# MaximEremenko/WebGPU-FFT

Measured on AMD Instinct MI355X. Metric: 1D c2c f32 GPoints/s at N=2^20 batch=4096, higher is better.
Workload: dtype f32

## Files before the change

webgpu-fft_amd/csrc/kern_regtile.hpp:

```cpp
#pragma once
#include "kern_xcd_real.hpp"
#include "kern_xcd_res.hpp"

namespace mi355 {

#ifndef MI355_RT_NT_OUT
#define MI355_RT_NT_OUT 0
#endif
#ifndef MI355_RT_EXP_SKIP_LAST
#define MI355_RT_EXP_SKIP_LAST 0
#endif
#ifndef MI355_RT_EXP_ALIGN
#define MI355_RT_EXP_ALIGN 0
#endif
#ifndef MI355_RT_EXP_ASC
#define MI355_RT_EXP_ASC 0
#endif
#ifndef MI355_RT_ONLY_PHASE
#define MI355_RT_ONLY_PHASE 0
#endif
#ifndef MI355_RT_NT_IN
#define MI355_RT_NT_IN MI355_XCD_NT
#endif
constexpr bool RT_NT_OUT = MI355_RT_NT_OUT != 0, RT_NT_IN = MI355_RT_NT_IN != 0;
// ... 305 lines not shown
#pragma unroll
        for (int q = 0; q < 16; ++q) rt_separate_store(wt, (unsigned)(32 + 64 * q), N2, wb[q], wb[31 - q]);
      }
      __syncthreads();
    }
    xcd_arrive(&f.ctl->bar[gslot][0]);
    if (!xcd_wait(&f.ctl->bar[gslot][0], (k + 1u) * gsize, f.spin_limit, f.sticky_error, &s_words[6])) return;
    cf* const po = f.out + tr * (f.out_pitch - MI355_RT_EXP_ALIGN);
    constexpr int sh = 0;
    for (unsigned tile = rank; tile < (MI355_RT_ONLY_PHASE == 1 ? 0u : (ROWS + 15) / 16 - MI355_RT_EXP_SKIP_LAST); tile += gsize) {
      cf v[64], v0[32], v1[32];
      const int r0 = (int)(tile * 16u) - sh;
      const int line = t >> 5, u = t & 31;
      {
        const int rr = r0 + line;
        const unsigned row = rr < 0 ? 0u : (rr < (int)ROWS ? (unsigned)rr : ROWS - 1);
        const cf* p = W + (size_t)row * N2 + u;
#pragma unroll
        for (int m = 0; m < 64; ++m) v[m] = p[32 * m];
        rt_fourstep(v, f, row, u);
      }
      rt_dft64(v, v0, v1);
      cf w[32];
      const int rl = t & 15, jj = t >> 4;
      const int k1s = r0 + rl;
      const unsigned k1 = (unsigned)k1s;
      const bool live = k1s >= 0 && k1s < (int)ROWS, edge = k1 == 0 || k1 == N1 / 2;
      rt_exchange_first(v0, v1, w, xb, line, u, rl, jj);
#pragma unroll
      for (int c = 0; c < 2; ++c) {
        const int j2 = jj + 32 * c;
        if (c == 1) rt_exchange_second(w, xb, rl, jj);
        rt_stage2(w, tw2, j2);
        if (f.scale != 1.0f) {
#pragma unroll
          for (int q = 0; q < 32; ++q) w[q] = w[q] * f.scale;
        }
        const unsigned kb = k1 + N1 * (unsigned)j2;
        if (live) {
#pragma unroll
          for (int q = 0; q < 16; ++q) st_stream<RT_NT_OUT>(po + (kb + (unsigned)(64 * q) * N1), w[q]);
        }
        if (live && !edge) {
#pragma unroll
          for (int q = 16; q < 32; ++q) { cf mm; mm.x = w[q].x; mm.y = -w[q].y; st_stream<RT_NT_OUT>(po + (NREAL - MI355_RT_EXP_ALIGN - (MI355_RT_EXP_ASC ? kb + 15u - 2u * (unsigned)rl : kb) - (unsigned)(64 * q) * N1), mm); }
        }
        if (c == 0 && k1 == 0 && jj == 0) st_stream<RT_NT_OUT>(po + NREAL / 2, w[16]);
      }
      __syncthreads();
    }
    if (!two_slots) {
      xcd_arrive(&f.ctl->bar[gslot][1]);
      if (!xcd_wait(&f.ctl->bar[gslot][1], (k + 1u) * gsize, f.spin_limit, f.sticky_error, &s_words[6])) return;
    }
  }
}
template <int N1_> struct XcdRtR2cCfgN { static constexpr int THREADS = RtCfg::THREADS, LDS_BYTES = XcdRtCfg<N1_, false>::LDS_BYTES; };

template <int N1_>
__global__ void __launch_bounds__(RtCfg::THREADS) fft_xcd_rt_c2r_kernel(const XcdFusedArgs f) {
  static_assert(N1_ == 2048 || N1_ == 1024, "2048 x 2048, or 1024 x 2048 with pass A on LDS-resident 16 x 1024 tiles (the packing then walks the LDS image)");
  using XC = XcdRtCfg<N1_, false>;
  using CA = typename XC::CA;
  MI_SMEM_DECL(smem);
  cf* xb = reinterpret_cast<cf*>(smem);
  cf* tw_a = xb + XC::DATA;
  cf* tw2 = tw_a + XC::TW_A;
  unsigned* s_words = reinterpret_cast<unsigned*>(tw2 + RtCfg::TW2_ELEMS);
  const int t = threadIdx.x;
  if constexpr (!XC::A_RT) { for (int i = t; i < XC::TW_A; i += RtCfg::THREADS) tw_a[i] = f.tw_a[i]; }
  for (int i = t; i < RtCfg::TW2_ELEMS; i += RtCfg::THREADS) tw2[i] = f.tw_b[i];
  if (!xcd_register(f.ctl, f.split, f.spin_limit, f.sticky_error, s_words)) return;
  const unsigned gslot = s_words[0], rank = s_words[1], gsize = s_words[2], gidx = s_words[4], groups = s_words[5];

  constexpr int N1 = N1_, N2 = 2048, COLS = N2 / 2 + 1;
  LineArgs aa{};
  aa.tw = f.tw_a; aa.num_tiles = (COLS + 15) / 16; aa.num_lines = COLS; aa.out_S = 16; aa.out_outer_stride = 0; aa.scale = 1.0f; aa.fs_group = 1;
  constexpr size_t wsize = (size_t)(N1 / 2) * N2;
  const bool two_slots = f.slots != 1u;
  cf* const W0 = f.wslots + (size_t)((two_slots ? 2u : 1u) * gslot) * wsize;
  const auto root = [&](unsigned m) { return cmul(f.tw_hi[m >> f.fs_shift], f.tw_lo[m & f.fs_lo_mask]); };
  unsigned k = 0;
  for (long long tr = gidx; tr < f.num_transforms; tr += groups, ++k) {
    cf* const W = W0 + (size_t)(two_slots ? (k & 1u) : 0u) * wsize;
    const cf* const X = f.in + tr * f.in_pitch;
    if constexpr (!XC::A_RT) {
      for (unsigned tile = rank; tile < (COLS + 15) / 16; tile += gsize) {
        cf v[CA::E];
        {
          const int line = t & 15, u = t >> 4;
          const int n2r = (int)(tile * 16u) + line, n2 = n2r > N2 / 2 ? N2 / 2 : n2r;
          const int up = u * N2 + n2;
          const int lo = n2 ? (N1 - 1 - u) * N2 + (N2 - n2) : (N1 - u) * N2;
#pragma unroll
          for (int q = 0; q < 32; ++q) {
            const int step = q * (N1 / 32) * N2;
            if (q < 16) { const cf x = X[up + step]; v[q] = cf{x.x, -x.y}; }
            else v[q] = X[lo - step];
          }
        }
        stage_compute_write<CA, 0>(v, aa, tile, t, xb, tw_a, nullptr);
        __syncthreads();
        stage_read<CA, 1>(v, aa, tile, t, xb);
        __syncthreads();
        stage_compute_write<CA, 1, false, true>(v, aa, tile, t, xb, tw_a, nullptr);
        __syncthreads();
        for (int p = t; p < (N1 / 2) * 16; p += RtCfg::THREADS) {
          const int i = p >> 4, c = p & 15;
          const int n2r = (int)(tile * 16u) + c;
          if (n2r > N2 / 2) continue;
          const cf a = cmul(xb[(2 * i) * 16 + c], root((unsigned)(2 * i) * (unsigned)n2r));
          const cf b = cmul(xb[(2 * i + 1) * 16 + c], root((unsigned)(2 * i + 1) * (unsigned)n2r));
          W[(size_t)i * N2 + n2r] = cf{a.x - b.y, a.y + b.x};
          if (n2r >= 1 && n2r < N2 / 2) W[(size_t)i * N2 + (N2 - n2r)] = cf{a.x + b.y, b.x - a.y};
        }
        __syncthreads();
      }
    } else
    for (unsigned tile = rank; tile < (COLS + 15) / 16; tile += gsize) {
      const int line = t & 15, i = t >> 4;
      cf v[64], v0[32], v1[32];
      const int n2r = (int)(tile * 16u) + line;
      const int n2 = n2r > N2 / 2 ? N2 / 2 : n2r;
      {
        const int up = i * N2 + n2;
        const int lo = n2 ? (N1 - 1 - i) * N2 + (N2 - n2) : (N1 - i) * N2;
#pragma unroll
        for (int m = 0; m < 32; ++m) { const cf x = X[up + (32 * m) * N2]; v[m] = cf{x.x, -x.y}; }
#pragma unroll
        for (int m = 32; m < 64; ++m) v[m] = X[lo - (32 * m) * N2];
      }
      rt_dft64(v, v0, v1);
      cf wa[32], wb[32];
      rt_exchange_first<true>(v0, v1, wa, xb, line, i, line, i);
      rt_stage2(wa, tw2, 2 * i);
      rt_exchange_second(wb, xb, line, i);
      rt_stage2(wb, tw2, 2 * i + 1);
      const bool live = n2r <= N2 / 2, mirror = live && n2r >= 1 && n2r < N2 / 2;
      const cf step = root(64u * (unsigned)n2);
      cf* const pd = W + (unsigned)i * N2 + (unsigned)n2;
      cf* const pm = W + (unsigned)i * N2 + (unsigned)(N2 - n2);
#pragma unroll
      for (int g = 0; g < 32; g += 8) {
        cf ra = root((unsigned)(2 * i + 64 * g) * (unsigned)n2), rb = root((unsigned)(2 * i + 1 + 64 * g) * (unsigned)n2);
#pragma unroll
        for (int q = g; q < g + 8; ++q) {
          const cf a = cmul(wa[q], ra), b = cmul(wb[q], rb);
          if (live) pd[(unsigned)(32 * q) * N2] = cf{a.x - b.y, a.y + b.x};
          if (mirror) pm[(unsigned)(32 * q) * N2] = cf{a.x + b.y, b.x - a.y};
          ra = cmul(ra, step); rb = cmul(rb, step);
        }
      }
      __syncthreads();
    }
    xcd_arrive(&f.ctl->bar[gslot][0]);
    if (!xcd_wait(&f.ctl->bar[gslot][0], (k + 1u) * gsize, f.spin_limit, f.sticky_error, &s_words[6])) return;
    cf* const y = f.out + tr * f.out_pitch;
    for (unsigned tile = rank; tile < (N1 / 2) / 16; tile += gsize) {
      cf v[64];
      rt_load_rows(v, W, tile * 16u, t);
      rt_finish_rows<false, RT_NT_OUT, false>(v, y, f, N1 / 2, tile * 16u, f.scale, t, xb, tw2, [](cf (&)[64]) {});
    }
    if (!two_slots) {
      xcd_arrive(&f.ctl->bar[gslot][1]);
      if (!xcd_wait(&f.ctl->bar[gslot][1], (k + 1u) * gsize, f.spin_limit, f.sticky_error, &s_words[6])) return;
    }
  }
}

#ifndef MI355_HX_WAVES
#define MI355_HX_WAVES 4
#endif
struct HxCfg {
  static constexpr int N = 1024, T = 16, THREADS = 512;
  static constexpr int HALF_ELEMS = T * 32 * 16;
  static constexpr int TW1_ELEMS = 31 * 32;
  static constexpr int LDS_BYTES = (HALF_ELEMS + TW1_ELEMS) * 8 + 64;
};

MI_DEV void hx_exchange(const cf (&v)[32], cf (&w)[32], cf* xb, int line, int u, int rl, int jj, bool first) {
  const int wb = u * 256 + ((line + u) & 15);
  const int rb = (jj & 15) * 16;
  if (first) {
#pragma unroll
    for (int q = 0; q < 16; ++q) xb[wb + q * 16] = v[q];
    __syncthreads();
#pragma unroll
    for (int uu = 0; uu < 32; ++uu) w[uu] = xb[uu * 256 + rb + ((rl + uu) & 15)];
    __syncthreads();
#pragma unroll
    for (int q = 0; q < 16; ++q) xb[wb + q * 16] = v[16 + q];
    __syncthreads();
    __syncthreads();
  } else {
#pragma unroll
    for (int q = 0; q < 16; ++q) xb[wb + q * 16] = v[q];
    __syncthreads();
    __syncthreads();
#pragma unroll
    for (int q = 0; q < 16; ++q) xb[wb + q * 16] = v[16 + q];
    __syncthreads();
#pragma unroll
    for (int uu = 0; uu < 32; ++uu) w[uu] = xb[uu * 256 + rb + ((rl + uu) & 15)];
    __syncthreads();
  }
}

template <bool INV>
__global__ void __launch_bounds__(HxCfg::THREADS, MI355_HX_WAVES) fft_xcd_hx_kernel(const XcdFusedArgs f) {
  MI_SMEM_DECL(smem);
  cf* xb = reinterpret_cast<cf*>(smem);
  cf* tw1 = xb + HxCfg::HALF_ELEMS;
  unsigned* s_words = reinterpret_cast<unsigned*>(tw1 + HxCfg::TW1_ELEMS);
  const int t = threadIdx.x;
  for (int i = t; i < HxCfg::TW1_ELEMS; i += HxCfg::THREADS) tw1[i] = f.tw_a[i];
  if (!xcd_register(f.ctl, f.split, f.spin_limit, f.sticky_error, s_words)) return;
  const unsigned gslot = s_words[0], rank = s_words[1], gsize = s_words[2], gidx = s_words[4], groups = s_words[5];
  constexpr unsigned N1 = 1024, N2 = 1024, NT = 64;
  const bool two_slots = f.slots != 1u;
  cf* const W0 = f.wslots + (size_t)((two_slots ? 2u : 1u) * gslot) * (size_t)f.N;
  const int cl = t & 15, cu = t >> 4;
  const int rl_ = t >> 5, ru = t & 31;
  const bool first = MI_UNIFORM_U32((unsigned)t >> 8) == 0u;
  const auto root = [&](unsigned m) { return cmul(f.tw_hi[m >> f.fs_shift], f.tw_lo[m & f.fs_lo_mask]); };
  unsigned k = 0;
  for (long long tr = gidx; tr < f.num_transforms; tr += groups, ++k) {
    cf* const W = W0 + (size_t)(two_slots ? (k & 1u) : 0u) * (size_t)f.N;
    const cf* const x = f.in + tr * f.in_pitch;
    for (unsigned tile = rank; tile < NT; tile += gsize) {
      cf v[32], w[32];
      {
        const cf* p = x + tile * 16u;
        const unsigned voff = (unsigned)cu * N2 + (unsigned)cl;
#pragma unroll
        for (int q = 0; q < 32; ++q) v[q] = cswap_if<INV>(ld_stream<RT_NT_IN>(sgpr_base(p + (unsigned)(32 * q) * N2) + voff));
      }
      fft_radix<32>(v);
      hx_exchange(v, w, xb, cl, cu, cl, cu, first);
      { int ti = cu; MI_OPAQUE_LANE_INT(ti);
#pragma unroll
      for (int q = 1; q < 32; ++q) w[q] = cmul(w[q], tw1[(q - 1) * 32 + ti]); }
      fft_radix<32>(w);
      cf* po = W + tile * 16u;
      const unsigned so = (unsigned)cu * N2 + (unsigned)cl;
#pragma unroll
      for (int q = 0; q < 32; ++q) *(sgpr_base(po + (unsigned)(32 * q) * N2) + so) = w[q];
    }
    xcd_arrive(&f.ctl->bar[gslot][0]);
    if (!xcd_wait(&f.ctl->bar[gslot][0], (k + 1u) * gsize, f.spin_limit, f.sticky_error, &s_words[6])) return;
    cf* const y = f.out + tr * f.out_pitch;
    for (unsigned tile = rank; tile < NT; tile += gsize) {
      cf v[32], w[32];
      {
        const unsigned k1 = tile * 16u + (unsigned)rl_;
        const cf* p = W + (size_t)(tile * 16u) * N2;
        const unsigned lo = (unsigned)rl_ * N2 + (unsigned)ru;
#pragma unroll
        for (int q = 0; q < 32; ++q) v[q] = *(sgpr_base(p + 32 * q) + lo);
        const cf step = root(k1 * 32u);
#pragma unroll
        for (int g = 0; g < 4; ++g) {
          cf r = root(k1 * (unsigned)(ru + 256 * g));
#pragma unroll
          for (int j = 0; j < 8; ++j) { v[8 * g + j] = cmul(v[8 * g + j], r); if (j < 7) r = cmul(r, step); }
        }
      }
      fft_radix<32>(v);
      hx_exchange(v, w, xb, rl_, ru, cl, cu, first);
      { int ti = cu; MI_OPAQUE_LANE_INT(ti);
#pragma unroll
      for (int q = 1; q < 32; ++q) w[q] = cmul(w[q], tw1[(q - 1) * 32 + ti]); }
      fft_radix<32>(w);
      cf* po = y + tile * 16u;
      const unsigned so = (unsigned)cu * N1 + (unsigned)cl;
#pragma unroll
      for (int q = 0; q < 32; ++q) {
        cf r = w[q];
        if (f.scale != 1.0f) r = r * f.scale;
        st_stream<XCD_NT>(sgpr_base(po + (unsigned)(32 * q) * N1) + so, cswap_if<INV>(r));
      }
    }
    if (!two_slots) {
      xcd_arrive(&f.ctl->bar[gslot][1]);
      if (!xcd_wait(&f.ctl->bar[gslot][1], (k + 1u) * gsize, f.spin_limit, f.sticky_error, &s_words[6])) return;
    }
  }
}

#ifndef MI355_RT1K_NT_OUT
#define MI355_RT1K_NT_OUT MI355_XCD_NT
#endif
#ifndef MI355_RT1K_NT_IN
#define MI355_RT1K_NT_IN MI355_RT_NT_IN
#endif
#ifndef MI355_RT1K_TW_FENCE
#define MI355_RT1K_TW_FENCE 8
#endif
#ifndef MI355_RT1K_PREFETCH
#define MI355_RT1K_PREFETCH 0
#endif
#ifndef MI355_RT1K_W_NT
#define MI355_RT1K_W_NT 0
#endif
template <int T_ = 32> struct Rt1kCfgT {
  static constexpr int N = 1024, T = T_, THREADS = 16 * T_;
  static constexpr int HALF_ELEMS = T * 32 * 16;
  static constexpr int TW1_ELEMS = 31 * 32;
  static constexpr int LDS_BYTES = (HALF_ELEMS + TW1_ELEMS) * 8 + 64;
};
using Rt1kCfg = Rt1kCfgT<32>;
template <int T = 32> MI_DEV int rt1k_slot(int line, int pl, int u) { return u * (16 * T) + pl * T + ((line + (u >> 1)) & (T - 1)); }

template <int T = 32, class Mid>
MI_DEV void rt1k_exchange(const cf (&va)[32], const cf (&vb)[32], cf (&w)[32], cf* xb, int line, int ua, int ub, int cl, int h, Mid&& mid) {
  const int wa = rt1k_slot<T>(line, 0, ua), wb2 = rt1k_slot<T>(line, 0, ub);
#pragma unroll
  for (int p = 0; p < 16; ++p) { xb[wa + p * T] = va[p]; xb[wb2 + p * T] = vb[p]; }
  __syncthreads();
#pragma unroll
  for (int uu = 0; uu < 32; ++uu) w[uu] = xb[uu * (16 * T) + h * T + ((cl + (uu >> 1)) & (T - 1))];
  __syncthreads();
#pragma unroll
  for (int p = 0; p < 16; ++p) { xb[wa + p * T] = va[16 + p]; xb[wb2 + p * T] = vb[16 + p]; }
  __syncthreads();
  MI_SCHED_FENCE();
  mid();
  MI_SCHED_FENCE();
#pragma unroll
  for (int uu = 0; uu < 32; ++uu) w[uu] = xb[uu * (16 * T) + h * T + ((cl + (uu >> 1)) & (T - 1))];
}

template <bool INV, int T = 32, bool VIEW = false, int N1_ = 1024>
__global__ void __launch_bounds__(Rt1kCfgT<T>::THREADS, 2) fft_xcd_rt1k_kernel(const XcdFusedArgs f) {
  using K = Rt1kCfgT<T>;
  static_assert(N1_ == 1024 || (N1_ == 2048 && T == 32 && !VIEW), "1024 x 1024, or 2048 x 1024 with pass A on 16 x 2048 register tiles");
  MI_SMEM_DECL(smem);
  cf* xb = reinterpret_cast<cf*>(smem);
  cf* tw1 = xb + K::HALF_ELEMS;
  cf* tw2 = tw1 + K::TW1_ELEMS;
  unsigned* s_words = reinterpret_cast<unsigned*>(tw2 + (N1_ == 2048 ? RtCfg::TW2_ELEMS : 0));
  const int t = threadIdx.x;
  for (int i = t; i < K::TW1_ELEMS; i += K::THREADS) tw1[i] = f.tw_b[i];
  if constexpr (N1_ == 2048) { for (int i = t; i < RtCfg::TW2_ELEMS; i += K::THREADS) tw2[i] = f.tw_a[i]; }
  if (!xcd_register(f.ctl, f.split, f.spin_limit, f.sticky_error, s_words)) return;
  const unsigned gslot = s_words[0], rank = s_words[1], gsize = s_words[2], gidx = s_words[4], groups = s_words[5];
  constexpr unsigned N1 = N1_, N2 = 1024, NT = N1 / T, TU = (unsigned)T;
  const bool two_slots = f.slots != 1u;
  cf* const W0 = f.wslots + (size_t)((two_slots ? 2u : 1u) * gslot) * (size_t)f.N;
  const int cl = t & (T - 1), h = t / T;
  const int rl = t >> 4, hh = t & 15;
  const auto root = [&](unsigned m) { return cmul(f.tw_hi[m >> f.fs_shift], f.tw_lo[m & f.fs_lo_mask]); };
  const auto stage1 = [&](cf (&w)[32], int j2) {
    int ti = j2; MI_OPAQUE_LANE_INT(ti);
#pragma unroll
    for (int q = 1; q < 32; ++q) {
      w[q] = cmul(w[q], tw1[(q - 1) * 32 + ti]);
      if (MI355_RT1K_TW_FENCE && q % MI355_RT1K_TW_FENCE == 0) MI_SCHED_FENCE();
    }
    fft_radix<32>(w);
  };
  unsigned k = 0;
  for (long long tr = gidx; tr < f.num_transforms; tr += groups, ++k) {
    cf* const W = W0 + (size_t)(two_slots ? (k & 1u) : 0u) * (size_t)f.N;
    const cf* const x = f.in + tr * f.in_pitch;
    if constexpr (N1_ == 2048) {
      for (unsigned tile = rank; tile < N2 / 16; tile += gsize) {
        cf v[64];
        rt_load_cols<INV, RT_NT_IN>(v, x, N2, tile * 16u, t);
        rt_finish_cols(v, W, N2, tile * 16u, t, xb, tw2, [](cf (&)[64]) {});
      }
    } else {
      cf va[32], vb[32], w[32];
      const unsigned voff = (unsigned)h * N2 + (unsigned)cl;
      constexpr int PF = MI355_RT1K_PREFETCH;
      const auto load_x = [&](const cf* p, unsigned row_uniform, unsigned tile) {
        if constexpr (VIEW) {
          const int i = (int)((row_uniform + (unsigned)h) * N2 + tile * TU + (unsigned)cl);
          const cf* const pe = p + row_uniform * N2 + voff;
          cf xv = {0.0f, 0.0f};
          if (i >= f.v_in_lo && i < f.v_in_hi) xv = *pe;
          return cswap_if<INV>(xv);
        } else return cswap_if<INV>(ld_stream<MI355_RT1K_NT_IN != 0>(sgpr_base(p + row_uniform * N2) + voff));
      };
      const auto load_a = [&](unsigned tile, int q0, int q1) {
        const cf* p = x + tile * TU;
#pragma unroll
        for (int q = 0; q < 32; ++q) if (q >= q0 && q < q1) va[q] = load_x(p, (unsigned)(32 * q), tile);
      };
      const auto load_b = [&](unsigned tile) {
        const cf* p = x + tile * TU;
#pragma unroll
        for (int q = 0; q < 32; ++q) vb[q] = load_x(p, (unsigned)(32 * q + 16), tile);
      };
      if (PF && rank < NT) load_a(rank, 0, PF);
      for (unsigned tile = rank; tile < NT; tile += gsize) {
        load_a(tile, PF, 32);
        load_b(tile);
        fft_radix<32>(va);
        fft_radix<32>(vb);
        cf* const po = W + tile * TU;
        const unsigned so = (unsigned)h * N2 + (unsigned)cl;
        rt1k_exchange<T>(va, vb, w, xb, cl, h, h + 16, cl, h, [&] {
          if (PF && tile + gsize < NT) load_a(tile + gsize, 0, PF);
          stage1(w, h);
#pragma unroll
          for (int q = 0; q < 32; ++q) st_stream<MI355_RT1K_W_NT != 0>(sgpr_base(po + (unsigned)(32 * q) * N2) + so, w[q]);
        });
        stage1(w, h + 16);
#pragma unroll
        for (int q = 0; q < 32; ++q) st_stream<MI355_RT1K_W_NT != 0>(sgpr_base(po + (unsigned)(32 * q + 16) * N2) + so, w[q]);
        __syncthreads();
      }
    }
    xcd_arrive(&f.ctl->bar[gslot][0]);
    if (!xcd_wait(&f.ctl->bar[gslot][0], (k + 1u) * gsize, f.spin_limit, f.sticky_error, &s_words[6])) return;
    cf* const y = f.out + tr * f.out_pitch;
    {
      cf va[32], vb[32], w[32];
      const unsigned lo = (unsigned)rl * N2 + 2u * (unsigned)hh;
      constexpr int PF = MI355_RT1K_PREFETCH / 2;
      const auto load_rows = [&](unsigned tile, int q0, int q1) {
        const cf* p = W + (size_t)(tile * TU) * N2;
#pragma unroll
        for (int q = 0; q < 32; ++q) if (q >= q0 && q < q1) {
          const cf4 pr = *reinterpret_cast<const cf4*>(sgpr_base(p + 32 * q) + lo);
          va[q] = cf{pr.x, pr.y}; vb[q] = cf{pr.z, pr.w};
        }
      };
      if (PF && rank < NT) load_rows(rank, 0, PF);
      for (unsigned tile = rank; tile < NT; tile += gsize) {
        load_rows(tile, PF, 32);
        {
          const unsigned k1 = tile * TU + (unsigned)rl;
          const cf step = root(k1 * 32u), one = root(k1);
#pragma unroll
          for (int g = 0; g < 4; ++g) {
            cf ra = root(k1 * (unsigned)(2 * hh + 256 * g));
            cf rb = cmul(ra, one);
#pragma unroll
            for (int j = 0; j < 8; ++j) {
              va[8 * g + j] = cmul(va[8 * g + j], ra); vb[8 * g + j] = cmul(vb[8 * g + j], rb);
              if (j < 7) { ra = cmul(ra, step); rb = cmul(rb, step); }
            }
          }
        }
        fft_radix<32>(va);
        fft_radix<32>(vb);
        cf* const po = y + tile * TU;
        const unsigned so = (unsigned)h * N1 + (unsigned)cl;
        const auto store = [&](cf (&ww)[32], unsigned off) {
#pragma unroll
          for (int q = 0; q < 32; ++q) {
            cf r = ww[q];
            if (f.scale != 1.0f) r = r * f.scale;
            if constexpr (VIEW) {
              const int kk = (int)(((unsigned)(32 * q) + off + (unsigned)h) * N1 + tile * TU + (unsigned)cl);
              cf* const pe = po + ((unsigned)(32 * q) + off) * N1 + so;
              if (kk < f.v_zlo || kk >= f.v_zhi) r = cf{0.0f, 0.0f};
              if (kk >= f.v_out_lo && kk < f.v_out_hi) *pe = cswap_if<INV>(r);
            } else st_stream<MI355_RT1K_NT_OUT != 0>(sgpr_base(po + ((unsigned)(32 * q) + off) * N1) + so, cswap_if<INV>(r));
          }
        };
        rt1k_exchange<T>(va, vb, w, xb, rl, 2 * hh, 2 * hh + 1, cl, h, [&] {
          if (PF && tile + gsize < NT) load_rows(tile + gsize, 0, PF);
          stage1(w, h); store(w, 0u);
        });
        stage1(w, h + 16);
        store(w, 16u);
        __syncthreads();
      }
    }
    if (!two_slots) {
      xcd_arrive(&f.ctl->bar[gslot][1]);
      if (!xcd_wait(&f.ctl->bar[gslot][1], (k + 1u) * gsize, f.spin_limit, f.sticky_error, &s_words[6])) return;
    }
  }
}

template <int N1_, bool VIEW = false>
__global__ void __launch_bounds__(Rt1kCfg::THREADS) fft_xcd_conv1m_kernel(const XcdFusedArgs f) {
  static_assert(N1_ == 1024, "1024 x 1024");
  MI_SMEM_DECL(smem);
  cf* xb = reinterpret_cast<cf*>(smem);
  cf* tw1 = xb + Rt1kCfg::HALF_ELEMS;
  unsigned* s_words = reinterpret_cast<unsigned*>(tw1 + Rt1kCfg::TW1_ELEMS);
  const int t = threadIdx.x;
  for (int i = t; i < Rt1kCfg::TW1_ELEMS; i += Rt1kCfg::THREADS) tw1[i] = f.tw_a[i];
  if (!xcd_register(f.ctl, f.split, f.spin_limit, f.sticky_error, s_words)) return;
  const unsigned gslot = s_words[0], rank = s_words[1], gsize = s_words[2], gidx = s_words[4], groups = s_words[5];
  constexpr unsigned N1 = 1024, N2 = 1024, NT = 32;
  cf* const Wg = f.wslots + (size_t)(2u * (f.slots ? f.slots : 1u) * gslot) * (size_t)f.N;
  const bool first = MI_UNIFORM_U32((unsigned)t >> 8) == 0u;
  const auto root = [&](unsigned m) { return cmul(f.tw_hi[m >> f.fs_shift], f.tw_lo[m & f.fs_lo_mask]); };
  const auto fresh = [&](int v) { if constexpr (VIEW) MI_OPAQUE_LANE_INT(v); return v; };
  const auto stage1 = [&](cf (&w)[32], int j2) {
    int ti = j2; MI_OPAQUE_LANE_INT(ti);
#pragma unroll
    for (int q = 1; q < 32; ++q) w[q] = cmul(w[q], tw1[(q - 1) * 32 + ti]);
    fft_radix<32>(w);
  };
  const auto load_rows = [&](cf (&va)[32], cf (&vb)[32], const cf* S, unsigned tile, int rl, int hh) {
    const unsigned k1 = tile * 32u + (unsigned)rl;
    const cf* p = S + (size_t)(tile * 32u) * N2;
    const unsigned lo = (unsigned)rl * N2 + 2u * (unsigned)hh;
#pragma unroll
    for (int q = 0; q < 32; ++q) {
      const cf4 pr = *reinterpret_cast<const cf4*>(sgpr_base(p + 32 * q) + lo);
      va[q] = cf{pr.x, pr.y}; vb[q] = cf{pr.z, pr.w};
    }
    const cf step = root(k1 * 32u), one = root(k1);
#pragma unroll
    for (int g = 0; g < 4; ++g) {
      cf ra = root(k1 * (unsigned)(2 * hh + 256 * g));
      cf rb = cmul(ra, one);
#pragma unroll
      for (int j = 0; j < 8; ++j) {
        va[8 * g + j] = cmul(va[8 * g + j], ra); vb[8 * g + j] = cmul(vb[8 * g + j], rb);
        if (j < 7) { ra = cmul(ra, step); rb = cmul(rb, step); }
      }
    }
  };
  unsigned vs1 = 0, vn1 = 0, vs2 = 0, vn2 = 0, vz_lo = 0, vz_n = 0, vshift = 0;
  if constexpr (VIEW) {
    const int sp = f.v_split, sh = f.v_shift, lo = f.v_out_lo, hi = f.v_out_hi;
    const int e1 = hi < sp ? hi : sp, b2 = lo > sp ? lo : sp;
    const int zl = f.v_zlo < sp ? f.v_zlo : f.v_zlo + sh, zh = f.v_zhi <= sp ? f.v_zhi : f.v_zhi + sh;
    vs1 = (unsigned)lo; vn1 = e1 > lo ? (unsigned)(e1 - lo) : 0u;
    vs2 = (unsigned)(b2 + sh); vn2 = hi > b2 ? (unsigned)(hi - b2) : 0u;
    vz_lo = (unsigned)zl; vz_n = zh > zl ? (unsigned)(zh - zl) : 0u;
    vshift = (unsigned)sh;
  }
  unsigned bar = 0;
  const auto group_barrier = [&]() -> bool {
    xcd_arrive(&f.ctl->bar[gslot][0]);
    ++bar;
    return xcd_wait(&f.ctl->bar[gslot][0], bar * gsize, f.spin_limit, f.sticky_error, &s_words[6]);
  };
  const unsigned L = f.slots ? f.slots : 1u;
  for (long long tr0 = (long long)gidx * L; tr0 < f.num_transforms; tr0 += (long long)groups * L) {
    const unsigned nl = (unsigned)(f.num_transforms - tr0 < (long long)L ? f.num_transforms - tr0 : (long long)L);
    for (unsigned tt = rank; tt < NT * nl; tt += gsize) {
      const unsigned ll = tt / NT, tile = tt - ll * NT;
      const cf* const x = f.in + (tr0 + ll) * f.in_pitch;
      cf* const W = Wg + (size_t)(2u * ll) * (size_t)f.N;
      const int ta = fresh(t), cl = ta & 31, h = ta >> 5;
      cf va[32], vb[32], w[32];
      {
        const cf* p = x + tile * 32u;
        const unsigned voff = (unsigned)h * N2 + (unsigned)cl;
        if constexpr (VIEW) {
          const unsigned rel = voff + tile * 32u - (unsigned)f.v_in_lo, span = (unsigned)(f.v_in_hi - f.v_in_lo);
#pragma unroll
          for (int q = 0; q < 32; ++q) {
            const cf* const pa = sgpr_base(p + (unsigned)(32 * q) * N2) + voff;
            const cf* const pb = sgpr_base(p + (unsigned)(32 * q + 16) * N2) + voff;
            va[q] = cf{0.0f, 0.0f}; vb[q] = cf{0.0f, 0.0f};
            if (rel + (unsigned)(32 * q) * N2 < span) va[q] = ld_stream<MI355_RT1K_NT_IN != 0>(pa);
            if (rel + (unsigned)(32 * q + 16) * N2 < span) vb[q] = ld_stream<MI355_RT1K_NT_IN != 0>(pb);
          }
        } else {
#pragma unroll
          for (int q = 0; q < 32; ++q) {
            va[q] = ld_stream<MI355_RT1K_NT_IN != 0>(sgpr_base(p + (unsigned)(32 * q) * N2) + voff);
            vb[q] = ld_stream<MI355_RT1K_NT_IN != 0>(sgpr_base(p + (unsigned)(32 * q + 16) * N2) + voff);
          }
        }
      }
      fft_radix<32>(va);
      fft_radix<32>(vb);
      cf* const po = W + tile * 32u;
      const unsigned so = (unsigned)h * N2 + (unsigned)cl;
      rt1k_exchange(va, vb, w, xb, cl, h, h + 16, cl, h, [&] {
        stage1(w, h);
#pragma unroll
        for (int q = 0; q < 32; ++q) *(sgpr_base(po + (unsigned)(32 * q) * N2) + so) = w[q];
      });
      stage1(w, h + 16);
#pragma unroll
      for (int q = 0; q < 32; ++q) *(sgpr_base(po + (unsigned)(32 * q + 16) * N2) + so) = w[q];
      __syncthreads();
    }
    if (!group_barrier()) return;
    for (unsigned kk = 0; kk < f.conv_k; ++kk) {
      const cf* const H = f.mul + (size_t)kk * (size_t)f.N;
      for (unsigned tt = rank; tt < 2 * NT * nl; tt += gsize) {
        const unsigned ll = tt / (2 * NT), tile = tt - ll * (2 * NT);
        const cf* const W = Wg + (size_t)(2u * ll) * (size_t)f.N;
        cf* const W2 = Wg + (size_t)(2u * ll + 1u) * (size_t)f.N;
        const int tm = fresh(t);
        const int ml = tm >> 5, mu = tm & 31;
        const int kl = tm & 15, ku = tm >> 4;
        cf v[32], w[32];
        {
          const unsigned k1 = tile * 16u + (unsigned)ml;
          const cf* p = W + (size_t)(tile * 16u) * N2;
          const unsigned lo = (unsigned)ml * N2 + (unsigned)mu;
#pragma unroll
          for (int q = 0; q < 32; ++q) v[q] = *(sgpr_base(p + 32 * q) + lo);
          const cf step = root(k1 * 32u);
#pragma unroll
          for (int g = 0; g < 4; ++g) {
            cf r = root(k1 * (unsigned)(mu + 256 * g));
#pragma unroll
            for (int j = 0; j < 8; ++j) { v[8 * g + j] = cmul(v[8 * g + j], r); if (j < 7) r = cmul(r, step); }
          }
        }
        fft_radix<32>(v);
        hx_exchange(v, w, xb, ml, mu, kl, ku, first);
        stage1(w, ku);
        {
          const cf* ph = H + tile * 16u;
          const unsigned ho = (unsigned)ku * N1 + (unsigned)kl;
#pragma unroll
          for (int q = 0; q < 32; ++q) {
            const cf hq = *(sgpr_base(ph + (unsigned)(32 * q) * N1) + ho);
            const cf pq = f.conv_conj ? cmul_conj(w[q], hq) : cmul(w[q], hq);
            v[q] = pq.yx;
          }
        }
        fft_radix<32>(v);
        hx_exchange(v, w, xb, kl, ku, kl, ku, first);
        stage1(w, ku);
        cf* const po = W2 + tile * 16u;
        const unsigned so = (unsigned)ku * N2 + (unsigned)kl;
#pragma unroll
        for (int q = 0; q < 32; ++q) *(sgpr_base(po + (unsigned)(32 * q) * N2) + so) = w[q];
      }
      if (!group_barrier()) return;
      for (unsigned tt = rank; tt < NT * nl; tt += gsize) {
        const unsigned ll = tt / NT, tile = tt - ll * NT;
        cf* const y = f.out + (tr0 + ll) * f.out_pitch + (long long)kk * f.out_kernel_pitch;
        const cf* const W2 = Wg + (size_t)(2u * ll + 1u) * (size_t)f.N;
        const int tc = fresh(t), cl = tc & 31, h = tc >> 5, rl = tc >> 4, hh = tc & 15;
        cf va[32], vb[32], w[32];
        load_rows(va, vb, W2, tile, rl, hh);
        fft_radix<32>(va);
        fft_radix<32>(vb);
        cf* const po = y + tile * 32u;
        const unsigned so = (unsigned)h * N1 + (unsigned)cl;
        const auto store = [&](cf (&ww)[32], unsigned off) {
#pragma unroll
          for (int q = 0; q < 32; ++q) st_stream<MI355_RT1K_NT_OUT != 0>(sgpr_base(po + ((unsigned)(32 * q) + off) * N1) + so, (ww[q] * f.scale).yx);
        };
        const auto store_view = [&](cf (&ww)[32], unsigned off) __attribute__((always_inline)) {
          const unsigned kb = so + tile * 32u;
#pragma unroll
          for (int q = 0; q < 32; ++q) {
            const unsigned ko = kb + ((unsigned)(32 * q) + off) * N1;
            cf r = (ww[q] * f.scale).yx;
            if (ko - vz_lo >= vz_n) r = cf{0.0f, 0.0f};
            const bool upper = ko - vs2 < vn2;
            cf* const pe = sgpr_base(po + ((unsigned)(32 * q) + off) * N1 - vshift) + (upper ? so : so + vshift);
            if (ko - vs1 < vn1 || upper) st_stream<MI355_RT1K_NT_OUT != 0>(pe, r);
          }
        };
        const auto put = [&](cf (&ww)[32], unsigned off) __attribute__((always_inline)) { if constexpr (VIEW) store_view(ww, off); else store(ww, off); };
        rt1k_exchange(va, vb, w, xb, rl, 2 * hh, 2 * hh + 1, cl, h, [&] { stage1(w, h); put(w, 0u); });
        stage1(w, h + 16);
        put(w, 16u);
        __syncthreads();
      }
      if (kk + 1 < f.conv_k) { if (!group_barrier()) return; }
    }
  }
}

}
```

webgpu-fft_amd/csrc/kern_xcd.hpp:

```cpp
#pragma once
#include "kern_lines.hpp"

#ifndef MI355_XCD_NT
#define MI355_XCD_NT 1
#endif

#ifndef MI355_XCD_W_NT_ST
#define MI355_XCD_W_NT_ST 0
#endif
#ifndef MI355_XCD_W_NT_LD
#define MI355_XCD_W_NT_LD 0
#endif

namespace mi355 {

constexpr bool XCD_NT = MI355_XCD_NT != 0;

struct XcdCtl {
  unsigned long long reg_packed;
  unsigned reg_pad[15];
  unsigned bar[512][16];
};

struct XcdFusedArgs {
  const cf* in;
  cf* out;
  cf* wslots;
  XcdCtl* ctl;
  unsigned* sticky_error;
  const cf* tw_a;
  const cf* tw_b;
  const cf* tw_lo;
  const cf* tw_hi;
  long long num_transforms;
  long long N;
  long long in_pitch, out_pitch;
  float scale;
  int fs_shift;
  unsigned fs_lo_mask;
  unsigned spin_limit;
  unsigned split;
  unsigned slots;
  unsigned solo;
  const cf* mul;
  unsigned conv_k, conv_conj;
  long long out_kernel_pitch;
  int v_in_lo, v_in_hi, v_out_lo, v_out_hi, v_zlo, v_zhi;
  int v_split, v_shift;
};

template <class C>
MI_DEV void fourstep_apply_chain(cf (&v)[C::E], const XcdFusedArgs& a, unsigned k1, int u) {
  using I = StageInfo<C, 0>;
  constexpr int NA = (I::R + 7) / 8;
  const auto root = [&](unsigned m) { return cmul(a.tw_hi[m >> a.fs_shift], a.tw_lo[m & a.fs_lo_mask]); };
  const cf step = root(k1 * (unsigned)(C::N / I::R));
#pragma unroll
  for (int b = 0; b < I::NB; ++b) {
    cf anchor[NA];
#pragma unroll
    for (int g = 0; g < NA; ++g) anchor[g] = root(k1 * (unsigned)(u + b * C::TPL + 8 * g * (C::N / I::R)));
#pragma unroll
    for (int g = 0; g < NA; ++g) {
      cf w = anchor[g];
#pragma unroll
      for (int j = 0; j < 8 && 8 * g + j < I::R; ++j) {
        cf& x = v[b * I::R + 8 * g + j];
        x = cmul(x, w);
        if (j < 7) w = cmul(w, step);
      }
    }
  }
}

#ifndef MI355_XCD_RELEASE
#define MI355_XCD_RELEASE 0
#endif
MI_DEV void xcd_arrive(unsigned* counter) {
  MI_WAIT_VMEM();
  __syncthreads();
  if (threadIdx.x == 0) {
#if MI355_XCD_RELEASE && !defined(MI355_HOST_EMU)
    __builtin_amdgcn_fence(__ATOMIC_RELEASE, "agent");
    MI_WAIT_VMEM();
#endif
    MI_ATOMIC_ADD_U32(counter, 1u);
  }
}
MI_DEV void xcd_local_handoff() {
  MI_WAIT_VMEM();
  __syncthreads();
  MI_ACQUIRE_AGENT();
}
#ifndef MI355_EXP_NO_WAIT
#define MI355_EXP_NO_WAIT 0
#endif
MI_DEV bool xcd_wait(unsigned* counter, unsigned target, unsigned spin_limit, unsigned* sticky, unsigned* s_flag) {
  if (threadIdx.x == 0) {
    unsigned ok = MI355_EXP_NO_WAIT;
    for (unsigned it = 0; it < spin_limit && !MI355_EXP_NO_WAIT; ++it) {
      if (MI_ATOMIC_LOAD_U32(counter) >= target) { ok = 1; break; }
      MI_SLEEP();
    }
    MI_ACQUIRE_AGENT();
    if (!ok) MI_ATOMIC_OR_U32(sticky, 2u);
    *s_flag = ok;
  }
  __syncthreads();
  return *s_flag != 0;
}

MI_DEV bool xcd_register(XcdCtl* ctl, unsigned split_arg, unsigned spin_limit, unsigned* sticky, unsigned* s_words) {
  if (threadIdx.x == 0) {
    const unsigned x = MI_XCC_ID() & 15u;
    unsigned ok = 0, r = 0;
    unsigned long long snap = 0;
    if (x < 8u && gridDim.x <= 8u * 255u) {
      const unsigned long long old = MI_ATOMIC_ADD_U64(&ctl->reg_packed, 1ull << (8u * x));
      r = (unsigned)(old >> (8u * x)) & 0xffu;
      if (r == 0xffu) MI_ATOMIC_OR_U32(sticky, 16u);
      for (unsigned it = 0; it < spin_limit; ++it) {
        snap = MI_ATOMIC_LOAD_U64(&ctl->reg_packed);
        unsigned total = 0;
        for (unsigned k = 0; k < 8; ++k) total += (unsigned)(snap >> (8u * k)) & 0xffu;
        if (total >= gridDim.x) { ok = 1; break; }
        MI_SLEEP();
      }
    }
    const unsigned split = split_arg ? split_arg : 1u;
    unsigned groups = 0, gi = 0, mine = 0, sub = 0, gsz = 0;
    for (unsigned k = 0; k < 8; ++k) {
      const unsigned cnt = (unsigned)(snap >> (8u * k)) & 0xffu;
      if (!cnt) continue;
      const unsigned per = (cnt + split - 1u) / split, nsub = (cnt + per - 1u) / per;
      if (k == x) {
        sub = r / per; mine = r - sub * per;
        gsz = (sub + 1u) * per <= cnt ? per : cnt - sub * per;
        gi = groups + sub;
      }
      groups += nsub;
    }
    s_words[0] = x * split + sub; s_words[1] = mine; s_words[2] = gsz; s_words[3] = ok; s_words[4] = gi; s_words[5] = groups;
    if (!ok) MI_ATOMIC_OR_U32(sticky, gridDim.x > 8u * 255u ? 16u : 1u);
  }
  __syncthreads();
  return s_words[3] != 0;
}

#ifndef MI355_XCD_PAIR
#define MI355_XCD_PAIR 1
#endif
template <class Cfg, bool PAIR_NT = true> struct PairOf {
  static constexpr int C = (MI355_XCD_PAIR && Cfg::T * 8 < 128) ? 128 / (Cfg::T * 8) : 1;
  static constexpr bool NT = XCD_NT && (C == 1 || PAIR_NT);
};
template <class C> MI_DEV long long xcd_tile(long long i, unsigned rank, unsigned gsize) {
  constexpr int P = PairOf<C>::C;
  return ((i / P) * (long long)gsize + rank) * P + (i % P);
}

template <class CA, class CB> struct XcdTables {
  static constexpr bool SHARED = CA::N == CB::N && CA::R0 == CB::R0 && CA::R1 == CB::R1 && CA::R2 == CB::R2;
  static constexpr int ELEMS = CA::TW_ELEMS + (SHARED ? 0 : CB::TW_ELEMS);
};

template <class CA, class CB, bool VIEW = false>
__global__ void __launch_bounds__(CA::THREADS) fft_xcd_fused_kernel(const XcdFusedArgs f) {
  static_assert(CA::THREADS == CB::THREADS, "both passes run in the same workgroup");
  static_assert(CA::IN_COL && CA::OUT_COL && !CB::IN_COL, "PASS_A, then PASS_B (four-step) or ROW (two-dimensional)");
  constexpr bool TWO_D = !CB::OUT_COL;
  MI_SMEM_DECL(smem);
  cf* lds = reinterpret_cast<cf*>(smem);
  constexpr int DATA = CA::DATA_ELEMS > CB::DATA_ELEMS ? CA::DATA_ELEMS : CB::DATA_ELEMS;
  using TB = XcdTables<CA, CB>;
  cf* tw_a = lds + DATA;
  cf* tw_b = TB::SHARED ? tw_a : tw_a + CA::TW_ELEMS;
  unsigned* s_words = reinterpret_cast<unsigned*>(tw_a + TB::ELEMS);
  const int t = threadIdx.x;
  for (int i = t; i < CA::TW_ELEMS; i += CA::THREADS) tw_a[i] = f.tw_a[i];
  if constexpr (!TB::SHARED) { for (int i = t; i < CB::TW_ELEMS; i += CA::THREADS) tw_b[i] = f.tw_b[i]; }

  if (f.solo) {
    if (t == 0) { s_words[0] = blockIdx.x; s_words[1] = 0; s_words[2] = 1; s_words[3] = 1; s_words[4] = blockIdx.x; s_words[5] = gridDim.x; }
    __syncthreads();
  } else if (!xcd_register(f.ctl, f.split, f.spin_limit, f.sticky_error, s_words)) return;
  const unsigned gslot = s_words[0], rank = s_words[1], gsize = s_words[2], gidx = s_words[4], groups = s_words[5];

  const long long N1 = CA::N, N2 = CB::N;
  LineArgs aa{}, ab{};
  aa.tw = f.tw_a; aa.num_tiles = N2 / CA::T; aa.num_lines = N2;
  aa.in_S = N2; aa.in_outer_stride = f.N; aa.out_S = N2; aa.out_outer_stride = f.N; aa.scale = 1.0f; aa.fs_group = 1;
  ab.tw = f.tw_b; ab.num_tiles = N1 / CB::T; ab.num_lines = N1;
  ab.in_S = 1; ab.in_outer_stride = N2; ab.out_S = TWO_D ? 1 : N1; ab.out_outer_stride = TWO_D ? N2 : f.N; ab.scale = f.scale; ab.fs_group = N1;
  if constexpr (VIEW) {
    static_assert(!TWO_D && CB::NSTAGES >= 2 && CB::NSTAGES <= 3, "rank-1 views of four-step lines");
    aa.v_in_lo = f.v_in_lo; aa.v_in_hi = f.v_in_hi; ab.v_out_lo = f.v_out_lo; ab.v_out_hi = f.v_out_hi; ab.v_zlo = f.v_zlo; ab.v_zhi = f.v_zhi;
  }
  const bool two_slots = f.slots != 1u && !f.solo;
  cf* const W0 = f.wslots + (size_t)((two_slots ? 2u : 1u) * gslot) * (size_t)f.N;
  unsigned k = 0;
  for (long long tr = gidx; tr < f.num_transforms; tr += groups, ++k) {
    cf* const W = W0 + (size_t)(two_slots ? (k & 1u) : 0u) * (size_t)f.N;
    aa.in = f.in + tr * f.in_pitch; aa.out = W;
    for (long long i = 0;; ++i) {
      const long long tile = xcd_tile<CA>(i, rank, gsize);
      if (tile - (i % PairOf<CA>::C) >= aa.num_tiles) break;
      if (tile >= aa.num_tiles) continue;
      cf v[CA::E];
      stage_read<CA, 0, PairOf<CA>::NT && !VIEW, VIEW>(v, aa, tile, t, lds);
      stage_compute_write<CA, 0>(v, aa, tile, t, lds, tw_a, nullptr);
      if constexpr (CA::NSTAGES >= 2) {
        __syncthreads();
        stage_read<CA, 1>(v, aa, tile, t, lds);
        __syncthreads();
        stage_compute_write<CA, 1, MI355_XCD_W_NT_ST != 0>(v, aa, tile, t, lds, tw_a, nullptr);
      }
      if constexpr (CA::NSTAGES == 3) {
        __syncthreads();
        stage_read<CA, 2>(v, aa, tile, t, lds);
        __syncthreads();
        stage_compute_write<CA, 2, MI355_XCD_W_NT_ST != 0>(v, aa, tile, t, lds, tw_a, nullptr);
      }
      __syncthreads();
    }
    if (f.solo) xcd_local_handoff();
    else {
      xcd_arrive(&f.ctl->bar[gslot][0]);
      if (!xcd_wait(&f.ctl->bar[gslot][0], (k + 1u) * gsize, f.spin_limit, f.sticky_error, &s_words[6])) return;
    }
    ab.in = W; ab.out = f.out + tr * f.out_pitch;
    for (long long i = 0;; ++i) {
      const long long tile = xcd_tile<CB>(i, rank, gsize);
      if (tile - (i % PairOf<CB>::C) >= ab.num_tiles) break;
      if (tile >= ab.num_tiles) continue;
      cf v[CB::E];
      stage_read<CB, 0, MI355_XCD_W_NT_LD != 0>(v, ab, tile, t, lds);
      if constexpr (!TWO_D) {
        int line, u; thread_map<CB, 0>(t, line, u);
        fourstep_apply_chain<CB>(v, f, (unsigned)(tile * CB::T + line), u);
      }
      stage_compute_write<CB, 0, PairOf<CB>::NT>(v, ab, tile, t, lds, tw_b, nullptr);
      if constexpr (CB::NSTAGES >= 2) {
        __syncthreads();
        stage_read<CB, 1>(v, ab, tile, t, lds);
        __syncthreads();
        stage_compute_write<CB, 1, PairOf<CB>::NT, false, false, VIEW && CB::NSTAGES == 2>(v, ab, tile, t, lds, tw_b, nullptr);
      }
      if constexpr (CB::NSTAGES == 3) {
        __syncthreads();
        stage_read<CB, 2>(v, ab, tile, t, lds);
        __syncthreads();
        stage_compute_write<CB, 2, PairOf<CB>::NT, false, false, VIEW>(v, ab, tile, t, lds, tw_b, nullptr);
      }
      __syncthreads();
    }
    if (f.solo) __syncthreads();
    else if (!two_slots) {
      xcd_arrive(&f.ctl->bar[gslot][1]);
      if (!xcd_wait(&f.ctl->bar[gslot][1], (k + 1u) * gsize, f.spin_limit, f.sticky_error, &s_words[6])) return;
    }
  }
}

template <class CA, class CB> struct XcdFusedCfg {
  static constexpr int DATA = CA::DATA_ELEMS > CB::DATA_ELEMS ? CA::DATA_ELEMS : CB::DATA_ELEMS;
  static constexpr int LDS_BYTES = (DATA + XcdTables<CA, CB>::ELEMS) * 8 + 64;
  static constexpr int THREADS = CA::THREADS;
  static_assert(LDS_BYTES <= 160 * 1024, "fused tile does not fit LDS");
};

}
```

Before: 197.9.

## Split second group barrier into early read-arrive and deferred wait; use packed-math complex multiply

Replaces the full arrive-and-wait barrier after pass B with a split handoff. Each workgroup signals that it has finished reading the workspace during its last pass-B tile, and the wait moves to just before the first pass-A store of the next transform, so pass-A loads and FFT overlap with the barrier. Complex multiplies in the twiddle and root paths are rewritten as inline v_pk_mul/v_pk_fma asm to cut VALU instructions. The output scale is now applied unconditionally and group words are marked uniform. The read-arrive fires before the workgroup's own reads have provably drained, which relies on the LDS exchange and syncthreads ordering for safety.

```diff
diff --git a/webgpu-fft_amd/csrc/kern_regtile.hpp b/webgpu-fft_amd/csrc/kern_regtile.hpp
--- a/webgpu-fft_amd/csrc/kern_regtile.hpp
+++ b/webgpu-fft_amd/csrc/kern_regtile.hpp
@@ -631,6 +631,12 @@
 #ifndef MI355_RT1K_W_NT
 #define MI355_RT1K_W_NT 0
 #endif
+#ifndef MI355_RT1K_SPLIT_HANDOFF
+#define MI355_RT1K_SPLIT_HANDOFF 1
+#endif
+#ifndef MI355_RT1K_LEAN_VALU
+#define MI355_RT1K_LEAN_VALU 1
+#endif
 template <int T_ = 32> struct Rt1kCfgT {
   static constexpr int N = 1024, T = T_, THREADS = 16 * T_;
   static constexpr int HALF_ELEMS = T * 32 * 16;
@@ -638,6 +644,16 @@
   static constexpr int LDS_BYTES = (HALF_ELEMS + TW1_ELEMS) * 8 + 64;
 };
 using Rt1kCfg = Rt1kCfgT<32>;
+MI_DEV cf rt1k_cmul(cf a, cf b) {
+#if MI355_RT1K_LEAN_VALU && !MI355_EXP_NO_MATH && !defined(MI355_HOST_EMU)
+  cf m, r;
+  asm("v_pk_mul_f32 %0, %1, %2 op_sel:[0,0] op_sel_hi:[0,1]" : "=v"(m) : "v"(a), "v"(b));
+  asm("v_pk_fma_f32 %0, %1, %2, %3 op_sel:[1,1,0] op_sel_hi:[1,0,1] neg_lo:[1,0,0]" : "=v"(r) : "v"(a), "v"(b), "v"(m));
+  return r;
+#else
+  return cmul(a, b);
+#endif
+}
 template <int T = 32> MI_DEV int rt1k_slot(int line, int pl, int u) { return u * (16 * T) + pl * T + ((line + (u >> 1)) & (T - 1)); }
 
 template <int T = 32, class Mid>
@@ -672,18 +688,19 @@
   for (int i = t; i < K::TW1_ELEMS; i += K::THREADS) tw1[i] = f.tw_b[i];
   if constexpr (N1_ == 2048) { for (int i = t; i < RtCfg::TW2_ELEMS; i += K::THREADS) tw2[i] = f.tw_a[i]; }
   if (!xcd_register(f.ctl, f.split, f.spin_limit, f.sticky_error, s_words)) return;
-  const unsigned gslot = s_words[0], rank = s_words[1], gsize = s_words[2], gidx = s_words[4], groups = s_words[5];
+  const unsigned gslot = MI_UNIFORM_U32(s_words[0]), rank = MI_UNIFORM_U32(s_words[1]), gsize = MI_UNIFORM_U32(s_words[2]), gidx = MI_UNIFORM_U32(s_words[4]), groups = MI_UNIFORM_U32(s_words[5]);
   constexpr unsigned N1 = N1_, N2 = 1024, NT = N1 / T, TU = (unsigned)T;
   const bool two_slots = f.slots != 1u;
+  constexpr bool SPLIT_HANDOFF = MI355_RT1K_SPLIT_HANDOFF && N1_ == 1024;
   cf* const W0 = f.wslots + (size_t)((two_slots ? 2u : 1u) * gslot) * (size_t)f.N;
   const int cl = t & (T - 1), h = t / T;
   const int rl = t >> 4, hh = t & 15;
-  const auto root = [&](unsigned m) { return cmul(f.tw_hi[m >> f.fs_shift], f.tw_lo[m & f.fs_lo_mask]); };
+  const auto root = [&](unsigned m) { return rt1k_cmul(f.tw_hi[m >> f.fs_shift], f.tw_lo[m & f.fs_lo_mask]); };
   const auto stage1 = [&](cf (&w)[32], int j2) {
     int ti = j2; MI_OPAQUE_LANE_INT(ti);
 #pragma unroll
     for (int q = 1; q < 32; ++q) {
-      w[q] = cmul(w[q], tw1[(q - 1) * 32 + ti]);
+      w[q] = rt1k_cmul(w[q], tw1[(q - 1) * 32 + ti]);
       if (MI355_RT1K_TW_FENCE && q % MI355_RT1K_TW_FENCE == 0) MI_SCHED_FENCE();
     }
     fft_radix<32>(w);
@@ -729,6 +746,9 @@
         fft_radix<32>(vb);
         cf* const po = W + tile * TU;
         const unsigned so = (unsigned)h * N2 + (unsigned)cl;
+        if (SPLIT_HANDOFF && !two_slots && k > 0 && tile == rank) {
+          if (!MI_UNIFORM_U32(xcd_wait<false>(&f.ctl->bar[gslot][1], k * gsize, f.spin_limit, f.sticky_error, &s_words[6], so == 0u))) return;
+        }
         rt1k_exchange<T>(va, vb, w, xb, cl, h, h + 16, cl, h, [&] {
           if (PF && tile + gsize < NT) load_a(tile + gsize, 0, PF);
           stage1(w, h);
@@ -765,11 +785,11 @@
 #pragma unroll
           for (int g = 0; g < 4; ++g) {
             cf ra = root(k1 * (unsigned)(2 * hh + 256 * g));
-            cf rb = cmul(ra, one);
+            cf rb = rt1k_cmul(ra, one);
 #pragma unroll
             for (int j = 0; j < 8; ++j) {
-              va[8 * g + j] = cmul(va[8 * g + j], ra); vb[8 * g + j] = cmul(vb[8 * g + j], rb);
-              if (j < 7) { ra = cmul(ra, step); rb = cmul(rb, step); }
+              va[8 * g + j] = rt1k_cmul(va[8 * g + j], ra); vb[8 * g + j] = rt1k_cmul(vb[8 * g + j], rb);
+              if (j < 7) { ra = rt1k_cmul(ra, step); rb = rt1k_cmul(rb, step); }
             }
           }
         }
@@ -781,7 +801,7 @@
 #pragma unroll
           for (int q = 0; q < 32; ++q) {
             cf r = ww[q];
-            if (f.scale != 1.0f) r = r * f.scale;
+            if (MI355_RT1K_LEAN_VALU || f.scale != 1.0f) r = r * f.scale;
             if constexpr (VIEW) {
               const int kk = (int)(((unsigned)(32 * q) + off + (unsigned)h) * N1 + tile * TU + (unsigned)cl);
               cf* const pe = po + ((unsigned)(32 * q) + off) * N1 + so;
@@ -792,6 +812,7 @@
         };
         rt1k_exchange<T>(va, vb, w, xb, rl, 2 * hh, 2 * hh + 1, cl, h, [&] {
           if (PF && tile + gsize < NT) load_rows(tile + gsize, 0, PF);
+          if (SPLIT_HANDOFF && !two_slots && tile + gsize >= NT) xcd_arrive_reads(&f.ctl->bar[gslot][1], so == 0u);
           stage1(w, h); store(w, 0u);
         });
         stage1(w, h + 16);
@@ -799,7 +820,7 @@
         __syncthreads();
       }
     }
-    if (!two_slots) {
+    if (!two_slots && !(SPLIT_HANDOFF && rank < NT)) {
       xcd_arrive(&f.ctl->bar[gslot][1]);
       if (!xcd_wait(&f.ctl->bar[gslot][1], (k + 1u) * gsize, f.spin_limit, f.sticky_error, &s_words[6])) return;
     }
diff --git a/webgpu-fft_amd/csrc/kern_xcd.hpp b/webgpu-fft_amd/csrc/kern_xcd.hpp
--- a/webgpu-fft_amd/csrc/kern_xcd.hpp
+++ b/webgpu-fft_amd/csrc/kern_xcd.hpp
@@ -87,6 +87,9 @@
     MI_ATOMIC_ADD_U32(counter, 1u);
   }
 }
+MI_DEV void xcd_arrive_reads(unsigned* counter, bool leader) {
+  if (leader) MI_ATOMIC_ADD_U32(counter, 1u);
+}
 MI_DEV void xcd_local_handoff() {
   MI_WAIT_VMEM();
   __syncthreads();
@@ -95,19 +98,24 @@
 #ifndef MI355_EXP_NO_WAIT
 #define MI355_EXP_NO_WAIT 0
 #endif
-MI_DEV bool xcd_wait(unsigned* counter, unsigned target, unsigned spin_limit, unsigned* sticky, unsigned* s_flag) {
-  if (threadIdx.x == 0) {
+template <bool ACQUIRE = true>
+MI_DEV bool xcd_wait(unsigned* counter, unsigned target, unsigned spin_limit, unsigned* sticky, unsigned* s_flag, bool leader) {
+  if (leader) {
     unsigned ok = MI355_EXP_NO_WAIT;
     for (unsigned it = 0; it < spin_limit && !MI355_EXP_NO_WAIT; ++it) {
       if (MI_ATOMIC_LOAD_U32(counter) >= target) { ok = 1; break; }
       MI_SLEEP();
     }
-    MI_ACQUIRE_AGENT();
+    if constexpr (ACQUIRE) MI_ACQUIRE_AGENT();
     if (!ok) MI_ATOMIC_OR_U32(sticky, 2u);
     *s_flag = ok;
   }
   __syncthreads();
   return *s_flag != 0;
+}
+
+MI_DEV bool xcd_wait(unsigned* counter, unsigned target, unsigned spin_limit, unsigned* sticky, unsigned* s_flag) {
+  return xcd_wait<true>(counter, target, spin_limit, sticky, s_flag, threadIdx.x == 0);
 }
 
 MI_DEV bool xcd_register(XcdCtl* ctl, unsigned split_arg, unsigned spin_limit, unsigned* sticky, unsigned* s_words) {
```

Result: faster. 205.8 (median of 6 runs) (+4.0%).
